# koadman/libMems

Measured on AMD Instinct MI355X. Metric: seed-mers/sec sorted+matched (+ MUMs/sec) at 1/2/4/8 MI355X; HBM GB/s vs roofline, higher is better.
Workload: dtype u64; 1 GPU; BASELINE config 3: 8 x 100 Mbp, seed weight 19 (0x7b974ef), MemHash seed stage (sorted+matched); genomes=8, genome_length=100000000, seedmers_total=799999792, seedmers_rank0=799999792, probes_rank0=100459493, parallelism=1 GPU

## Files before the change

libmems_amd/csrc/groups.hip:

```cpp
#include <cstdlib>
#include <type_traits>

#include "match_device.h"
#include "seed_device.h"

namespace mums {

namespace {

constexpr int kGTile = kSegTile;
constexpr int kGRounds = kGTile / kBlock;
constexpr int kSlots = kGTile / 2;
#ifndef MUMS_GROUP_SPLIT
#define MUMS_GROUP_SPLIT 2
#endif
constexpr int kGSplit = MUMS_GROUP_SPLIT;
constexpr int kGSub = kGTile / kGSplit;
constexpr int kGSubRounds = kGSub / kBlock;
constexpr int kSubSlots = kGSub / 2;
static_assert(kGSub % kBlock == 0 && kGSubRounds * (kBlock / 64) <= 64, "probe sub-tile");

__device__ __forceinline__ uint32_t blk_excl_scan(uint32_t v, uint32_t* s_w, uint32_t* total) {
    const int lane = threadIdx.x & 63, wv = threadIdx.x >> 6;
    uint32_t inc = v;
    #pragma unroll
    for (int d = 1; d < 64; d <<= 1) {
        uint32_t t = __shfl_up(inc, d, 64);
        if (lane >= d) inc += t;
    }
    if (lane == 63) s_w[wv] = inc;
    __syncthreads();
// ... 134 lines not shown
                                                                double inv_table) {
    constexpr int kGRounds = kGSubRounds;
    constexpr int kWaves = kBlock / 64;
    __shared__ uint64_t srec[kGSub];
    __shared__ uint16_t heads[kSubSlots];
    __shared__ uint32_t wcnt[kGRounds * kWaves];
    __shared__ uint32_t s_w[2][kWaves];
    __shared__ uint32_t s_ng[kWaves];
    __shared__ uint32_t s_red[2];
    __shared__ uint64_t s_prev, s_next;
    __shared__ uint8_t s_gl[256];
    __shared__ uint32_t s_gb[kMaxG + 1];
    const int lane = threadIdx.x & 63;
    const int wv = __builtin_amdgcn_readfirstlane(threadIdx.x >> 6);
    const SegTile td = tiles[blockIdx.x / kGSplit];
    const uint32_t part0 = (blockIdx.x % kGSplit) * (uint32_t)kGSub;
    if (td.count <= part0) {
        if (threadIdx.x == 0) {
            tile_count[blockIdx.x] = 0;
            tile_count[gridDim.x + 32 + blockIdx.x] = 0;
        }
        return;
    }
    const uint64_t tile0 = td.start + part0;
    const uint32_t cnt = td.count - part0 < (uint32_t)kGSub ? td.count - part0 : (uint32_t)kGSub;

    uint32_t kx[kGRounds];
    {
        uint64_t x[kGRounds];
        #pragma unroll
        for (int r = 0; r < kGRounds; ++r) {
            const uint32_t q = r * kBlock + threadIdx.x;
            x[r] = rec[tile0 + (q < cnt ? q : cnt - 1)];
        }
        #pragma unroll
        for (int r = 0; r < kGRounds; ++r) {
            const uint32_t q = r * kBlock + threadIdx.x;
            if (q < cnt) srec[q] = x[r];
            kx[r] = (uint32_t)(x[r] >> (IB + 1));
        }
// ... 137 lines not shown
                                                               const uint32_t* __restrict__ tile_off,
                                                               const uint64_t* __restrict__ slot_info,
                                                               const uint32_t* __restrict__ slot_bucket,
                                                               uint64_t* __restrict__ probe_info,
                                                               uint32_t* __restrict__ probe_bucket,
                                                               uint32_t slots_per_block) {
    const uint32_t n = tile_count[blockIdx.x];
    const uint64_t o = tile_off[blockIdx.x];
    const uint64_t sb = (uint64_t)blockIdx.x * slots_per_block;
    for (uint32_t k = threadIdx.x; k < n; k += kBlock) {
        probe_info[o + k] = slot_info[sb + k];
        probe_bucket[o + k] = slot_bucket[sb + k];
    }
}

__global__ void flat_tiles_kernel(uint64_t N, uint64_t nt, SegTile* __restrict__ tiles) {
    const uint64_t t = (uint64_t)blockIdx.x * blockDim.x + threadIdx.x;
    if (t >= nt) return;
    SegTile d{};
    d.start = t * kGTile;
    d.bstart = 0;
    d.bend = N;
    const uint64_t rem = N - d.start;
    d.count = (uint32_t)(rem < (uint64_t)kGTile ? rem : (uint64_t)kGTile);
    d.hbase = 0;
    d.ntb = (uint32_t)nt;
    d.tb = (uint32_t)t;
    tiles[t] = d;
}

#ifndef MUMS_MAT_WIDE
#define MUMS_MAT_WIDE 1
#endif
constexpr bool kMatWide = MUMS_MAT_WIDE != 0;
struct __attribute__((aligned(8))) Rec2 { uint64_t a, b; };

template <int MG, typename View, bool kGl = false>
__global__ __launch_bounds__(kBlock) void probe_materialize_kernel(View v, const uint64_t* __restrict__ probe_info,
                                                                   uint64_t P, GenomeTable gt, MatchParams mp, int L,
// ... 356 lines not shown
    hipLaunchKernelGGL(row_bucket_kernel, dim3((unsigned)((P + kBlock - 1) / kBlock)), dim3(kBlock), 0, st, rows, P, G,
                       table_size, 1.0 / (double)table_size, d_bounds, nranks, out);
    return hipGetLastError();
}

hipError_t launch_gather_rows(const int64_t* src, const uint32_t* perm, uint64_t P, int G, int64_t* dst,
                              hipStream_t st) {
    if (P == 0) return hipSuccess;
    const uint64_t n = P * (uint64_t)(G + 1);
    const uint64_t per = (uint64_t)kBlock * kGatherIPT;
    hipLaunchKernelGGL(gather_rows_ilp_kernel, dim3((unsigned)((n + per - 1) / per)), dim3(kBlock), 0, st, src, perm, n,
                       (uint32_t)(G + 1), dst);
    return hipGetLastError();
}

hipError_t launch_flat_tiles(uint64_t N, SegTile* d_tiles, hipStream_t st) {
    const uint64_t nt = (N + kGTile - 1) / kGTile;
    if (nt == 0) return hipSuccess;
    hipLaunchKernelGGL(flat_tiles_kernel, dim3((unsigned)((nt + 255) / 256)), dim3(256), 0, st, N, nt, d_tiles);
    return hipGetLastError();
}

template <int MG, typename View>
hipError_t launch_probe_tiles(View v, const SegTile* tiles, uint64_t ntiles, uint64_t N, const GenomeTable& gt,
                              const MatchParams& mp, int L, uint32_t* tile_count, uint64_t* slot_info,
                              uint32_t* slot_bucket, void* counters, hipStream_t st) {
    if (ntiles == 0) return hipSuccess;
    if constexpr (RecIB<View>::value > 0) {
        const bool fast = mp.repeat_tol == 0 && mp.enum_tol == 1;
        const double inv_t = 1.0 / (double)mp.table_size;
        if (RecIB<View>::value == 32 && gt.gl_n > 0 && fast && !getenv("MUMS_DEV_PROBE_GENERAL"))
            hipLaunchKernelGGL((probe_tile_rec_kernel<MG, RecIB<View>::value, true, true>),
                               dim3((unsigned)(ntiles * kGSplit)), dim3(kBlock), 0, st, v.rec, tiles, gt, mp, L,
                               tile_count, slot_info, slot_bucket, (DevCounters*)counters, inv_t);
// ... 74 lines not shown
```

libmems_amd/csrc/mums_capi.hip:

```cpp
#include <hip/hip_runtime.h>

#include <algorithm>
#include <array>
#include <chrono>
#include <functional>
#include <cstddef>
#include <cstdio>
#include <cstdlib>
#include <cstring>
#include <memory>
#include <string>
#include <vector>

#include "../../include/mums.h"
#include "match_device.h"
#include "mums_internal.h"
#include "seed_device.h"

using namespace mums;

namespace {

struct DevBuf {
    void* p = nullptr;
// ... 767 lines not shown
        HIPCHK(ctx->ctab.ensure(64));
        HIPCHK(hipMemsetAsync(ctx->ctab.p, 0, 64, st));
        HIPCHK(launch_seed_scatter_chunk(ctx->ss, lgt, ctx->packed.as<uint32_t>(), B, hist, T, 0, 0, out, st,
                                         ctx->ctab.as<uint64_t>(), B));
    }
    HIPCHK(seg_bucket_starts(B > 0 ? hist : nullptr, T, B, n, bstart, st));
    return MUMS_OK;
}

void records_live(mums_ctx* ctx) {
    for (DevBuf* b : {&ctx->rowtmp, &ctx->sids, &ctx->summ, &ctx->chain_tmp}) b->drop_view();
}

int ensure_merge_space(mums_ctx* ctx, uint64_t n, int mb, int key_bits, ProbeSpace* ps) {
    records_live(ctx);
    const uint64_t ub = seg_tiles_upper(n, mb);
    HIPCHK(ctx->recA.ensure(n * 8 + 64));
    HIPCHK(ctx->recB.ensure(n * 8 + 64));
    HIPCHK(ctx->tiles.ensure(ub * sizeof(SegTile) + 64));
    HIPCHK(ctx->mstart.ensure(((1ull << mb) + 64) * 4));
    size_t tmpb = std::max(seg_tmp_bytes(n, mb), onesweep_tmp_bytes(n, mb, key_bits));
    tmpb = std::max(tmpb, std::max(scan_tmp_bytes(n), radix_tmp_bytes(n / 2 + 1)));
    tmpb = std::max(tmpb, scan_tmp_bytes((uint64_t)ctx->table_size));
    HIPCHK(ctx->tmp.ensure(tmpb));
    return ensure_probe_space(ctx, n, ub, ps);
}

int tie_fix_stream(mums_ctx* ctx, const RsStream& s, uint64_t n, hipStream_t st);
bool wants_tie_order(const mums_ctx* ctx);

int merge_stage(mums_ctx* ctx, uint64_t n, int mb, int key_bits, const MatchParams& mp, const ProbeSpace& ps,
                hipStream_t st, int ib = 32, uint64_t* rA = nullptr, uint64_t* rB = nullptr) {
    DevCounters* dc = ctx->counters.as<DevCounters>();
    if (!rA) rA = ctx->recA.as<uint64_t>();
    if (!rB) rB = ctx->recB.as<uint64_t>();
    SegTile* tiles = ctx->tiles.as<SegTile>();
    const uint32_t* bstart = ctx->mstart.as<uint32_t>();
    const uint64_t ub = seg_tiles_upper(n, mb);
    const bool prof = ctx->profiling;
    HIPCHK(build_seg_tiles_from_starts(bstart, mb, n, tiles, &dc->ntiles, ctx->tmp.p, st));
    int buf = 0;
    if (ib != 32 && !(n < (1ull << 30) && key_bits <= 32))
        return fail(ctx, MUMS_E_UNSUPPORTED, "33-bit records need < 2^30 records per merge");
    const bool mask_parity = mp.repeat_tol == 0 && mp.enum_tol == 1;
    ctx->parity_masked = false;
    const bool onesweep = ctx->use_onesweep && n < (1ull << 30) && key_bits <= 32;
    const bool wide = onesweep && mask_parity && ib == 32 && seg_wide_sort_enabled() && seg_wide_passes(key_bits) <= 3;
    if (wide) {
        HIPCHK(seg_onesweep_sort_wide(rA, rB, n, key_bits, mb, bstart, ctx->tmp.p, &dc->err, &buf, st,
                                      prof ? ctx->ev_ds : nullptr, 32));
        ctx->parity_masked = true;
    } else if (onesweep) {
        HIPCHK(seg_onesweep_sort(rA, rB, n, key_bits, mb, bstart, ctx->tmp.p, &dc->err, &buf, st,
                                 prof ? ctx->ev_ds : nullptr, ib, mask_parity));
        ctx->parity_masked = mask_parity && seg_onesweep_launches(key_bits) < (key_bits + 7) / 8;
    } else
        HIPCHK(seg_radix_sort(rA, rB, n, key_bits, tiles, ub, ctx->tmp.p, &buf, st, prof ? ctx->ev_ds : nullptr));
    ctx->sorted_buf = buf;
    ctx->sorted_rec = buf ? rB : rA;
    ctx->sort_passes = wide ? seg_wide_passes(key_bits) : onesweep ? seg_onesweep_launches(key_bits) : (key_bits + 7) / 8;
    HIPCHK(hipEventRecord(ctx->ev[EV_SORT], st));
    if (wants_tie_order(ctx) && ib == 32 && !ctx->shard) {
        RsStream s{};
        s.kind = 0;
        s.rec = ctx->sorted_rec;
        s.bstart = bstart;
        s.B = mb;
        s.kbits = 2 * ctx->w + 1;
        const int rc = tie_fix_stream(ctx, s, n, st);
        if (rc) return rc;
    }
    if (ib == 33)
// ... 273 lines not shown
        s.B = B;
        s.kbits = 2 * ctx->w + 1;
        uint64_t* dst = ctx->sorted_buf ? ctx->recA.as<uint64_t>() : ctx->recB.as<uint64_t>();
        if (ctx->parity_masked) {
            HIPCHK(seg_parity_fix(const_cast<uint64_t*>(ctx->sorted_rec), dst, N, s.kbits - B, B, ctx->mstart.as<uint32_t>(), ctx->tmp.p,
                                  &dc->err, st));
            ctx->parity_masked = false;
        }
        HIPCHK(ctx->rsbst.ensure(((1ull << B) + 64) * 4));
        rc = restart_fixup(ctx, s, N, dst, nullptr, ctx->rsbst.as<uint32_t>(), &nl, &changed, st);
        if (rc || !changed) return rc;
        HIPCHK(hipMemcpyAsync(ctx->mstart.p, ctx->rsbst.p, ((1ull << B) + 1) * 4, hipMemcpyDeviceToDevice, st));
        ctx->sorted_buf ^= 1;
        ctx->sorted_rec = dst;
        SegTile* tiles = ctx->tiles.as<SegTile>();
        HIPCHK(build_seg_tiles_from_starts(ctx->mstart.as<uint32_t>(), B, nl, tiles, &dc->ntiles, ctx->tmp.p, st));
        HIPCHK(hipMemsetAsync(&dc->repeat_limit, 0, 8, st));
        rc = groups_dispatch<RecView>(ctx, RecView{dst}, tiles, seg_tiles_upper(nl, B), mp, ps.probe_info,
                                      ps.probe_bucket, ps.slot_info, ps.slot_bucket, st);
    } else {
        const size_t kb = ctx->key64 ? 8 : 4;
        (void)kb;
        s.kind = ctx->key64 ? 2 : 1;
        s.key = ctx->sorted_key;
        s.idx = ctx->sorted_idx;
        void* dk = ctx->sorted_buf ? ctx->kA.p : ctx->kB.p;
        uint32_t* dv = ctx->sorted_buf ? ctx->vA.as<uint32_t>() : ctx->vB.as<uint32_t>();
        rc = restart_fixup(ctx, s, N, dk, dv, nullptr, &nl, &changed, st);
        if (rc || !changed) return rc;
        ctx->sorted_buf ^= 1;
        ctx->sorted_key = dk;
        ctx->sorted_idx = dv;
        SegTile* tiles = ctx->tiles.as<SegTile>();
// ... 327 lines not shown
    const int kbits = 2 * ctx->w + 1;
    int gbits = 0;
    while ((1 << gbits) < G) ++gbits;
    if (kbits + gbits > 63) return fail(ctx, MUMS_E_UNSUPPORTED, "ParallelMemHash compat: seed weight too large");
    ctx->packed_path = false;
    ctx->key64 = true;
    ctx->msd_bits = 0;
    ctx->progress.clear();
    const uint64_t kmask = (1ull << kbits) - 1;

    uint64_t words = 0;
    const uint32_t T = layout_packed(gt, &words);
    HIPCHK(ctx->packed.ensure(words * 4 + 64));
    HIPCHK(ctx->counters.ensure(sizeof(DevCounters)));
    DevCounters* dc = ctx->counters.as<DevCounters>();
    const uint64_t ntiles_groups = (N + kSegTile - 1) / kSegTile;
    HIPCHK(ctx->ckey.ensure(N * 8 + 64));
    HIPCHK(ctx->kA.ensure(N * 8 + 64));
    HIPCHK(ctx->kB.ensure(N * 8 + 64));
    HIPCHK(ctx->vA.ensure(N * 4 + 64));
    HIPCHK(ctx->vB.ensure(N * 4 + 64));
    HIPCHK(ctx->cval.ensure(enum_rows ? 2 * (N + 64) * 4 : N * 4 + 64));
    HIPCHK(ctx->tiles.ensure(ntiles_groups * sizeof(SegTile) + 64));
    size_t tmpb = std::max(scan_tmp_bytes(N + 1), radix_tmp_bytes(N + 1));
    tmpb = std::max(tmpb, scan_tmp_bytes((uint64_t)ctx->table_size));
    HIPCHK(ctx->tmp.ensure(tmpb));
    ProbeSpace ps{};
    int rc = ensure_probe_space(ctx, N, ntiles_groups, &ps);
    if (rc) return rc;

    int mx = -1;
// ... 263 lines not shown
        HIPCHK(hipEventRecord(ctx->ev[EV_BUCKETS], st));
        ctx->stage_done = MUMS_STAGE_SEEDS;
        if (stage >= MUMS_STAGE_ALL) {
            rc = find_tail(ctx, mp, ctx->packed.as<uint32_t>(), [&](MatProbes* v) {
                v->rows = ctx->mprobe.as<int64_t>();
                return MUMS_OK;
            }, st);
            if (rc) return rc;
        }
        HIPCHK(hipStreamSynchronize(st));
        HIPCHK(hipMemcpy(&ctx->hc, dc, sizeof(DevCounters), hipMemcpyDeviceToHost));
        fill_stats(ctx, N);
        return MUMS_OK;
    }
    SegTile* tiles = ctx->tiles.as<SegTile>();
    HIPCHK(launch_flat_tiles(n_live, tiles, st));
    if (ctx->compat_rec)
        rc = groups_dispatch<RecView>(ctx, RecView{ctx->sorted_rec}, tiles, (n_live + kSegTile - 1) / kSegTile, mp,
                                      ps.probe_info, ps.probe_bucket, ps.slot_info, ps.slot_bucket, st);
    else
        rc = groups_dispatch<PairView<uint64_t>>(
            ctx, PairView<uint64_t>{(const uint64_t*)ctx->sorted_key, ctx->sorted_idx}, tiles,
            (n_live + kSegTile - 1) / kSegTile, mp, ps.probe_info, ps.probe_bucket, ps.slot_info, ps.slot_bucket, st);
    if (rc) return rc;
    rc = finish_seeds(ctx, ps, st, stage >= MUMS_STAGE_ALL);
    if (rc) return rc;
    ctx->compat_pfirst.clear();
    if (ctx->match_log) {
        DevBuf pf;
        HIPCHK(pf.ensure(((uint64_t)nch + 1) * 4 + 64));
        HIPCHK(launch_compat_probe_chunks(ctx->probe_info, ctx->P, (const uint64_t*)ctx->sorted_key, kbits, nch,
                                          pf.as<uint32_t>(), st));
        ctx->compat_pfirst.resize((size_t)nch + 1);
// ... 148 lines not shown
    if (!s) return fail(ctx, MUMS_E_INVALID, "null stream");
    if (ctx->own_stream && ctx->stream) (void)hipStreamDestroy(ctx->stream);
    ctx->stream = (hipStream_t)s;
    ctx->own_stream = false;
    return MUMS_OK;
}

int mums_set_seed(mums_ctx* ctx, uint64_t pattern) {
    if (check_ctx(ctx)) return MUMS_E_INVALID;
    ctx->seed = pattern;
    return MUMS_OK;
}

int mums_set_params(mums_ctx* ctx, uint32_t repeat_tol, uint32_t enum_tol, uint32_t table_size) {
    if (check_ctx(ctx)) return MUMS_E_INVALID;
    if (table_size == 0 || table_size > 0x7FFFFFFFu)
        return fail(ctx, MUMS_E_INVALID, "table size must be in [1, 2^31)");
    ctx->repeat_tol = repeat_tol;
    ctx->enum_tol = enum_tol;
    ctx->table_size = table_size;
    return MUMS_OK;
}

int mums_set_mask(mums_ctx* ctx, int masked, uint64_t seq_mask) {
    if (check_ctx(ctx)) return MUMS_E_INVALID;
    ctx->masked = masked ? 1 : 0;
    ctx->seq_mask = seq_mask;
    return MUMS_OK;
}

int mums_add_genome(mums_ctx* ctx, const char* ascii, uint64_t n) {
    if (check_ctx(ctx)) return MUMS_E_INVALID;
// ... 853 lines not shown
    const auto chunks = shard_key_chunks(bst, ctx->shard_kcount, shard_chunk_cap());
    if (chunks.empty() && ctx->shard_kcount)
        return fail(ctx, MUMS_E_UNSUPPORTED, "one MSD bucket holds more than 2^30 records");
    DevCounters* dc = ctx->counters.as<DevCounters>();
    const MatchParams mp{ctx->repeat_tol, ctx->enum_tol, ctx->table_size, ctx->masked, ctx->seq_mask};
    const size_t W = (size_t)(G + 1) * 8;
    uint64_t P_total = 0, groups = 0;
    ctx->fused_keys = false;
    for (const auto& ch : chunks) {
        const uint32_t b0 = ch.first, b1 = ch.second;
        const uint64_t o = bst[b0], nc = (uint64_t)bst[b1] - o;
        std::vector<uint32_t> sub(nbk + 1);
        for (uint32_t b = 0; b <= nbk; ++b) sub[b] = b < b0 ? 0u : (b < b1 ? bst[b] - (uint32_t)o : (uint32_t)nc);
        HIPCHK(hipMemcpyAsync(ctx->mstart.p, sub.data(), sub.size() * 4, hipMemcpyHostToDevice, st));
        SegTile* tiles = ctx->tiles.as<SegTile>();
        HIPCHK(build_seg_tiles_from_starts(ctx->mstart.as<uint32_t>(), mb, nc, tiles, &dc->ntiles, ctx->tmp.p, st));
        const uint64_t ub = seg_tiles_upper(nc, mb);
        int rc;
        if (ctx->rec_ib == 33)
            rc = groups_dispatch<RecViewT<33>>(ctx, RecViewT<33>{rec + o}, tiles, ub, mp, ps.probe_info,
                                               ps.probe_bucket, ps.slot_info, ps.slot_bucket, st);
        else
            rc = groups_dispatch<RecView>(ctx, RecView{rec + o}, tiles, ub, mp, ps.probe_info, ps.probe_bucket,
                                          ps.slot_info, ps.slot_bucket, st);
        if (rc) return rc;
        rc = finish_seeds(ctx, ps, st);
        if (rc) return rc;
        const uint64_t Pc = ctx->P;
        if (rows && Pc) {
            if (P_total + Pc >= (1ull << 32) - 64)
                return fail(ctx, MUMS_E_UNSUPPORTED, "more than 2^32 seed probes on one rank");
            if (ctx->rowsall.cap < (P_total + Pc + 1) * W) {
// ... 63 lines not shown
    if (pw && ib33) HIPCHK(launch_pairwise_emit(v64, n, ctx->gt, ctx->L, ncalls, off, rows, st));
    else if (pw) HIPCHK(launch_pairwise_emit(v, n, ctx->gt, ctx->L, ncalls, off, rows, st));
    else if (ib33) HIPCHK(launch_enum_emit(v64, n, ctx->gt, mp, ctx->L, ncalls, off, P, rows, st));
    else HIPCHK(launch_enum_emit(v, n, ctx->gt, mp, ctx->L, ncalls, off, P, rows, st));
    HIPCHK(hipStreamSynchronize(st));
    ctx->P = P;
    ctx->st.probes = P;
    ctx->shard_rows_built = true;
    return MUMS_OK;
}

int shard_chunk_rows(mums_ctx* ctx, hipStream_t st) {
    if (!shard_rows_from_all(ctx) || ctx->shard_rows_built) return MUMS_OK;
    if (ctx->enum_tol > 1 || ctx->pairwise) return shard_enum_rows(ctx, st);
    ProbeSpace ps{};
    int rc = ensure_probe_space(ctx, ctx->shard_n, seg_tiles_upper(ctx->shard_n, ctx->shard_mb), &ps);
    if (rc) return rc;
    HIPCHK(hipMemsetAsync(ctx->counters.p, 0, sizeof(DevCounters), st));
    rc = shard_groups_chunked(ctx, const_cast<uint64_t*>(ctx->sorted_rec), ctx->shard_bst, ps, true, st);
    if (rc) return rc;
    ctx->shard_rows_built = true;
    return MUMS_OK;
}

int shard_regroup(mums_ctx* ctx, uint64_t* dst, uint64_t nl, const std::vector<uint32_t>& bst, const ProbeSpace& ps,
                  uint64_t restarts, const uint64_t* offset_log, hipStream_t st) {
    const int mb = ctx->shard_mb;
    ctx->sorted_buf ^= 1;
    ctx->sorted_rec = dst;
    DevCounters* dc = ctx->counters.as<DevCounters>();
    const uint64_t rep = ctx->hc.repeat_limit;
// ... 9 lines not shown
        const uint64_t P = ctx->P, groups = ctx->st.groups;
        ctx->hc.repeat_limit = rep;
        ctx->restarts = restarts;
        ctx->offset_log.assign(offset_log, offset_log + restarts * (uint64_t)ctx->gt.G);
        ctx->shard_restart_pending = false;
        shard_merge_stats(ctx, nl);
        ctx->P = P;
        ctx->st.probes = P;
        ctx->st.groups = groups;
        return MUMS_OK;
    }
    HIPCHK(hipMemcpyAsync(ctx->mstart.p, bst.data(), bst.size() * 4, hipMemcpyHostToDevice, st));
    ctx->live_n = nl;
    ctx->live_bst = bst;
    SegTile* tiles = ctx->tiles.as<SegTile>();
    HIPCHK(build_seg_tiles_from_starts(ctx->mstart.as<uint32_t>(), mb, nl, tiles, &dc->ntiles, ctx->tmp.p, st));
    HIPCHK(hipMemsetAsync(&dc->repeat_limit, 0, 8, st));
    const MatchParams mp{ctx->repeat_tol, ctx->enum_tol, ctx->table_size, ctx->masked, ctx->seq_mask};
    const uint64_t ub = seg_tiles_upper(nl, mb);
    int rc;
    if (ctx->rec_ib == 33)
        rc = groups_dispatch<RecViewT<33>>(ctx, RecViewT<33>{dst}, tiles, ub, mp, ps.probe_info, ps.probe_bucket,
                                           ps.slot_info, ps.slot_bucket, st);
    else
        rc = groups_dispatch<RecView>(ctx, RecView{dst}, tiles, ub, mp, ps.probe_info, ps.probe_bucket, ps.slot_info,
                                      ps.slot_bucket, st);
    if (rc) return rc;
    rc = finish_seeds(ctx, ps, st);
    if (rc) return rc;
    HIPCHK(h2d_sync(&dc->repeat_limit, &rep, 8, ctx->stream));
    ctx->hc.repeat_limit = rep;
    ctx->restarts = restarts;
    ctx->offset_log.assign(offset_log, offset_log + restarts * (uint64_t)ctx->gt.G);
    ctx->shard_restart_pending = false;
// ... 1780 lines not shown
        HIPCHK(hipEventRecord(ctx->ev[EV_CHAINS], st));
        uint32_t* bstart = ctx->mstart.as<uint32_t>();
        if (!resident) {
            HIPCHK(exclusive_scan_u32(slice, (uint64_t)nbc8 * T, ctx->tmp.p, nullptr, st));
            HIPCHK(launch_seed_scatter_chunk(ctx->ss, gt, ctx->packed.as<uint32_t>(), B, slice, T, dlo, nbc8, rA, st));
        }
        if (live_rec) {
            n_c = n_live[c];
            HIPCHK(hipMemcpyAsync(bstart, lbst.as<uint32_t>() + (uint64_t)c * (nbc + 1), (nbc + 1) * 4ull,
                                  hipMemcpyDeviceToDevice, st));
        } else {
            rc = chunk_starts(c, n_c, bstart);
            if (rc) return rc;
        }
        SegTile* tiles = ctx->tiles.as<SegTile>();
        const uint64_t ub = seg_tiles_upper(n_c, mb);
        HIPCHK(build_seg_tiles_from_starts(bstart, mb, n_c, tiles, &dc->ntiles, ctx->tmp.p, st));
        if (!resident) {
            int buf = 0;
            HIPCHK(seg_onesweep_sort(rA, rB, n_c, 31, mb, bstart, ctx->tmp.p, &dc->err, &buf, st,
                                     prof ? ctx->ev_ds : nullptr, 33, mp.repeat_tol == 0 && mp.enum_tol == 1));
            ctx->sorted_rec = buf ? rB : rA;
            if (prof)
                for (int p = 0; p < npass; ++p) {
                    float ms = 0.f;
                    (void)hipEventElapsedTime(&ms, ctx->ev_ds[2 * p], ctx->ev_ds[2 * p + 1]);
                    ms_dom += ms;
                }
            dom_bytes += n_c * 16 * (uint64_t)npass;
            dom_launches += (uint64_t)npass;
        } else {
            ctx->sorted_rec = live_rec ? live_rec + o : (sbuf ? rB : rA);
// ... 646 lines not shown
```

libmems_amd/csrc/mums_internal.h:

```cpp
#pragma once

#include <hip/hip_runtime.h>
#include <stdint.h>
#include <stdlib.h>

#include <vector>

#include "restart_plan.h"

namespace mums {

constexpr int kMaxG = 64;
constexpr int kRepeatLimit = 1000;
constexpr int kBlock = 256;
#ifndef MUMS_SEED_TILE
#define MUMS_SEED_TILE 4096
#endif
constexpr int kSeedTile = MUMS_SEED_TILE;
#ifndef MUMS_SEG_TILE
#define MUMS_SEG_TILE 4096
#endif
constexpr int kSegTile = MUMS_SEG_TILE;
constexpr int kLocalIPT = 16;
constexpr int kMaxMsdBits = 11;
constexpr int kMaxSegBucketBits = 12;

constexpr int kMaxSeedRuns = 16;

struct SeedSpec {
    uint64_t pattern;
    int L;
    int w;
    int nruns;
    int run_start[32];
    int run_len[32];
    int run_dst[32];
    int run_sh[kMaxSeedRuns];
// ... 158 lines not shown
                             const uint32_t* d_bstart, void* d_tmp, uint32_t* d_err, int* out_buf, hipStream_t st,
                             hipEvent_t* ev_ds = nullptr, int key_shift = 32, bool mask_parity = false,
                             bool key_runs = false, const uint32_t* hist_in = nullptr,
                             const uint64_t* gsrc = nullptr, uint32_t* gout = nullptr);
size_t seg_parity_fix_tmp_bytes(uint64_t n);
hipError_t seg_parity_fix(uint64_t* rec, uint64_t* scratch, uint64_t n, int key_bits, int msd_bits,
                          const uint32_t* d_bstart, void* d_tmp, uint32_t* d_err, hipStream_t st, int key_shift = 32);
int seg_onesweep_launches(int key_bits);
bool seg_wide_sort_enabled();
int seg_wide_passes(int key_bits);
size_t onesweep_wide_tmp_bytes(uint64_t n, int msd_bits, int key_bits);
hipError_t seg_onesweep_sort_wide(uint64_t* recA, uint64_t* recB, uint64_t n, int key_bits, int msd_bits,
                                  const uint32_t* d_bstart, void* d_tmp, uint32_t* d_err, int* out_buf,
                                  hipStream_t st, hipEvent_t* ev_ds, int key_shift = 32);

uint64_t group_slot_count(uint64_t ntiles);
uint64_t group_blocks(uint64_t ntiles, bool packed);
template <int MG, typename View>
hipError_t launch_probe_tiles(View v, const SegTile* tiles, uint64_t ntiles, uint64_t N, const GenomeTable& gt,
                              const MatchParams& mp, int L, uint32_t* tile_count, uint64_t* slot_info,
                              uint32_t* slot_bucket, void* counters, hipStream_t st);
hipError_t launch_probe_compact(uint64_t nblocks, const uint32_t* tile_count, const uint32_t* tile_off,
                                const uint64_t* slot_info, const uint32_t* slot_bucket, uint64_t* probe_info,
                                uint32_t* probe_bucket, hipStream_t st, bool packed);
hipError_t launch_bucket_records(const uint32_t* b, uint64_t P, uint64_t* rec, hipStream_t st);
hipError_t launch_bucket_split(const uint64_t* rec, uint64_t P, uint32_t* b, uint32_t* ids, hipStream_t st);
template <int MG, typename View>
hipError_t launch_materialize(View v, const uint64_t* probe_info, uint64_t P, const GenomeTable& gt,
                              const MatchParams& mp, int L, int64_t* rows, hipStream_t st, uint64_t* lkey = nullptr,
                              uint32_t* fsk = nullptr, uint32_t* lhash = nullptr, int32_t* rows32 = nullptr);
// ... 7 lines not shown
                              int kb_rec, uint64_t* key, uint64_t* idx, hipStream_t st);
hipError_t launch_chain_dest(const uint32_t* fk, uint64_t nch, const uint32_t* pdest, uint32_t* cdest, hipStream_t st);
hipError_t launch_inverse_perm(const uint32_t* perm, uint64_t n, uint32_t* inv, hipStream_t st);
hipError_t launch_chain_tags(const uint32_t* chain_of, const uint32_t* perm, const uint32_t* sdest, uint64_t P,
                             const uint32_t* cinv, const uint32_t* cstart, uint32_t* tags, hipStream_t st);
hipError_t launch_chain_entries_out(const int64_t* pool, const uint32_t* fk, const uint32_t* cperm,
                                    const uint32_t* scdest, uint64_t nch, int G, const uint32_t* pinv,
                                    const uint32_t* rstart, int64_t* eout, uint32_t* fout, hipStream_t st);
hipError_t launch_kept_dest(const int64_t* rows, uint64_t P, int G, const uint32_t* chain_of, const uint32_t* cinv,
                            const uint2* thr, const uint32_t* fk, const uint32_t* pdest, uint32_t nranks, uint32_t* dest,
                            hipStream_t st);
hipError_t launch_dest_first(const uint32_t* sdest, uint64_t P, uint32_t* first, hipStream_t st);
hipError_t launch_entry_first(const uint32_t* scdest, uint64_t nch, const uint32_t* rcount, const uint32_t* perm,
                              const uint32_t* sdest, uint64_t K, const uint32_t* chain_of, const uint32_t* cinv,
                              const uint32_t* rstart, uint32_t* efirst, hipStream_t st);
hipError_t launch_flat_tiles(uint64_t N, SegTile* d_tiles, hipStream_t st);

hipError_t launch_bucket_ranges(const uint32_t* sb, uint64_t P, uint32_t* bstart, uint32_t* bend, uint32_t* d_max,
                                hipStream_t st);
template <int MG, typename View>
hipError_t launch_replay_kept(View v, const GenomeTable& gt, const MatchParams& mp, int L, uint64_t P,
                              const int64_t* pool, const uint32_t* chain_of, const uint32_t* fk, uint32_t nch,
                              void* d_tmp, void* d_radix_tmp, void* d_scan_tmp, uint32_t lds_cap, uint32_t* tsize,
                              void* ctr, uint64_t* dbg, hipStream_t st, uint64_t* mlog, uint32_t** tbl_out,
                              const uint32_t** base_out, void* (*alloc)(void*, size_t), void* alloc_ctx,
                              const uint32_t* jl = nullptr);
}
struct mums_ctx;
namespace mums {
hipStream_t ctx_stream(mums_ctx* ctx);
int ctx_device(mums_ctx* ctx);
// ... 256 lines not shown
```

libmems_amd/csrc/seed_device.h:

```cpp
#pragma once

#include "mums_internal.h"

namespace mums {

__device__ __forceinline__ uint32_t xcd_grouped_block(uint32_t b, uint32_t n) {
    const uint32_t q = n >> 3, r = n & 7u, x = b & 7u;
    return (x < r ? x * (q + 1) : r * (q + 1) + (x - r) * q) + (b >> 3);
}

__device__ __forceinline__ uint64_t revcomp2w(uint64_t v, int w) {
    uint64_t x = ~v;
    x = __builtin_bitreverse64(x);
    x = ((x >> 1) & 0x5555555555555555ull) | ((x & 0x5555555555555555ull) << 1);
    return x >> (64 - 2 * w);
}

__device__ __forceinline__ uint64_t ckey_finish(uint64_t v, int w) {
    const uint64_t rc = revcomp2w(v, w);
    const uint64_t par = rc < v ? 1ull : 0ull;
    return ((par ? rc : v) << 1) | par;
}

__device__ __forceinline__ uint64_t ckey_from_mer(uint64_t mer, const SeedSpec& ss) {
// ... 60 lines not shown
__device__ __forceinline__ uint32_t ckey_top_static(uint64_t mer) {
    constexpr SeedRuns R = seed_runs(PAT);
    constexpr int B = (K + 1) / 2;
    static_assert(K >= 1 && 2 * B <= 2 * R.w && 2 * B <= 32, "top digit wider than the seed");
    uint64_t v = 0;
    #pragma unroll
    for (int r = 0; r < R.n; ++r) v |= (R.sh[r] >= 0 ? (mer >> R.sh[r]) : (mer << -R.sh[r])) & R.mask[r];
    const uint32_t ft = (uint32_t)(v >> (2 * R.w - K));
    const uint32_t lowc = ~(uint32_t)v & (uint32_t)((1ull << (2 * B)) - 1);
    uint32_t rr = __builtin_bitreverse32(lowc) >> (32 - 2 * B);
    rr = ((rr >> 1) & 0x55555555u) | ((rr & 0x55555555u) << 1);
    const uint32_t rt = rr >> (2 * B - K);
    return ft < rt ? ft : rt;
}

constexpr uint64_t kSeedW15 = 0x7ac9afull;
constexpr uint64_t kSeedW19 = 0x7b974efull;
constexpr uint64_t kSeedW21 = 0x7ddaddfull;

__device__ __forceinline__ uint64_t window_at(const uint32_t* __restrict__ W, uint64_t p) {
    const uint64_t wi = p >> 4;
    const int sh = 2 * (int)(p & 15);
    const uint64_t hi = ((uint64_t)W[wi] << 32) | W[wi + 1];
    const uint64_t lo = W[wi + 2];
    return (hi << sh) | ((lo << sh) >> 32);
}

__device__ __forceinline__ uint64_t ckey_at(const uint32_t* __restrict__ W, uint64_t p, const SeedSpec& ss) {
    return ckey_from_mer(window_at(W, p), ss);
}
// ... 41 lines not shown
```

libmems_amd/csrc/seeds.hip:

```cpp
#include <cstdlib>
#include <type_traits>

#include "seed_device.h"

namespace mums {

namespace {

constexpr int kTile = kSeedTile;
constexpr int kPerThread = kTile / kBlock;
constexpr int kHalo = 32;
constexpr int kTileBytes = kTile + kHalo;
constexpr int kTileWords = kTileBytes / 16 + 3;
constexpr int kWaves = kBlock / 64;

struct AsciiPtrs { const char* p[kMaxG]; };

template <uint64_t PAT>
constexpr int kStaticMsd = PAT == 0 ? 0 : (2 * seed_runs(PAT).w + 1 > 32 ? 2 * seed_runs(PAT).w + 1 - 32 : 0);

__device__ __forceinline__ uint32_t dna2(uint32_t c) {
    const uint32_t lc = c | 0x20u;
    const uint32_t one = (lc == 'c') | (lc == 'b') | (lc == 'y');
    const uint32_t two = (lc == 'g') | (lc == 's') | (lc == 'k');
// ... 91 lines not shown
    {
        const uint64_t pw = packed_words(n);
        uint32_t* out = packed + gt.woff[g];
        for (int k = tid; k < kTile / 16 + 2; k += kBlock) {
            const uint64_t wi = (uint64_t)x * (kTile / 16) + k;
            if ((k < kTile / 16 || p0 + kTile >= n) && wi < pw) out[wi] = words[k];
        }
    }

    if (kMode == 1 && nb <= 1) return;
    const uint64_t base = gt.base[g];
    const int klow = 2 * ss.w + 1 - msd_bits;
    if constexpr (kMode == 1 && PAT != 0 && kStaticMsd<PAT> >= 1 && kStaticMsd<PAT> <= kMaxMsdBits) {
        constexpr int kTop = kStaticMsd<PAT> > 8 ? 8 : kStaticMsd<PAT>;
        if (msd_bits == kTop) {
            #pragma unroll 4
            for (int j = 0; j < kPerThread; ++j) {
                const int q = tid + j * kBlock;
                const uint64_t p = p0 + (uint64_t)q;
                if (p >= m) break;
                const int wi = q >> 4, sh = 2 * (q & 15);
                const uint64_t hi = ((uint64_t)words[wi] << 32) | words[wi + 1];
                const uint64_t lo = words[wi + 2];
                atomicAdd(&bh[ckey_top_static<PAT, kTop>((hi << sh) | ((lo << sh) >> 32))], 1u);
            }
            __syncthreads();
            for (int i = tid; i < nb; i += kBlock) hist[(uint64_t)i * T + t] = bh[i];
            return;
        }
    }
// ... 369 lines not shown
```

Baseline: 37.32 billion seed-mers/s.

## Decouple probe tile take from staging size and add register-field top-key histogram

Probe workgroups now consume a configurable slice (kProbeTake, default 1984) rather than the full staged half-tile. Tile builders, upper bounds and flat tiles take a separate probe tile size, and the radix-sort path rebuilds sort-sized tiles before rebuilding probe tiles. A new specialized MSD histogram path extracts the top-bit canonical key from two 32-bit register fields using alignbit per thread, processing 16 contiguous positions per thread instead of strided word loads. The aim is less per-seed extraction work in the histogram and better probe-tile balance and occupancy, at the cost of more tiles, extra tile rebuilds and layout-dependent correctness risk. The table size bound is also relaxed to allow 2^31.

```diff
diff --git a/libmems_amd/csrc/groups.hip b/libmems_amd/csrc/groups.hip
--- a/libmems_amd/csrc/groups.hip
+++ b/libmems_amd/csrc/groups.hip
@@ -11,10 +11,8 @@
 constexpr int kGTile = kSegTile;
 constexpr int kGRounds = kGTile / kBlock;
 constexpr int kSlots = kGTile / 2;
-#ifndef MUMS_GROUP_SPLIT
-#define MUMS_GROUP_SPLIT 2
-#endif
-constexpr int kGSplit = MUMS_GROUP_SPLIT;
+constexpr int kGSplit = kProbeSplit;
+constexpr int kGTake = kProbeTake;
 constexpr int kGSub = kGTile / kGSplit;
 constexpr int kGSubRounds = kGSub / kBlock;
 constexpr int kSubSlots = kGSub / 2;
@@ -179,7 +177,7 @@
     const int lane = threadIdx.x & 63;
     const int wv = __builtin_amdgcn_readfirstlane(threadIdx.x >> 6);
     const SegTile td = tiles[blockIdx.x / kGSplit];
-    const uint32_t part0 = (blockIdx.x % kGSplit) * (uint32_t)kGSub;
+    const uint32_t part0 = (blockIdx.x % kGSplit) * (uint32_t)kGTake;
     if (td.count <= part0) {
         if (threadIdx.x == 0) {
             tile_count[blockIdx.x] = 0;
@@ -188,7 +186,7 @@
         return;
     }
     const uint64_t tile0 = td.start + part0;
-    const uint32_t cnt = td.count - part0 < (uint32_t)kGSub ? td.count - part0 : (uint32_t)kGSub;
+    const uint32_t cnt = td.count - part0 < (uint32_t)kGTake ? td.count - part0 : (uint32_t)kGTake;
 
     uint32_t kx[kGRounds];
     {
@@ -356,15 +354,15 @@
     }
 }
 
-__global__ void flat_tiles_kernel(uint64_t N, uint64_t nt, SegTile* __restrict__ tiles) {
+__global__ void flat_tiles_kernel(uint64_t N, uint64_t nt, uint32_t tile, SegTile* __restrict__ tiles) {
     const uint64_t t = (uint64_t)blockIdx.x * blockDim.x + threadIdx.x;
     if (t >= nt) return;
     SegTile d{};
-    d.start = t * kGTile;
+    d.start = t * tile;
     d.bstart = 0;
     d.bend = N;
     const uint64_t rem = N - d.start;
-    d.count = (uint32_t)(rem < (uint64_t)kGTile ? rem : (uint64_t)kGTile);
+    d.count = (uint32_t)(rem < (uint64_t)tile ? rem : (uint64_t)tile);
     d.hbase = 0;
     d.ntb = (uint32_t)nt;
     d.tb = (uint32_t)t;
@@ -751,10 +749,11 @@
     return hipGetLastError();
 }
 
-hipError_t launch_flat_tiles(uint64_t N, SegTile* d_tiles, hipStream_t st) {
-    const uint64_t nt = (N + kGTile - 1) / kGTile;
+hipError_t launch_flat_tiles(uint64_t N, SegTile* d_tiles, hipStream_t st, bool packed) {
+    const uint32_t tile = (uint32_t)(packed ? kProbeTile : kGTile);
+    const uint64_t nt = (N + tile - 1) / tile;
     if (nt == 0) return hipSuccess;
-    hipLaunchKernelGGL(flat_tiles_kernel, dim3((unsigned)((nt + 255) / 256)), dim3(256), 0, st, N, nt, d_tiles);
+    hipLaunchKernelGGL(flat_tiles_kernel, dim3((unsigned)((nt + 255) / 256)), dim3(256), 0, st, N, nt, tile, d_tiles);
     return hipGetLastError();
 }
 
diff --git a/libmems_amd/csrc/mums_capi.hip b/libmems_amd/csrc/mums_capi.hip
--- a/libmems_amd/csrc/mums_capi.hip
+++ b/libmems_amd/csrc/mums_capi.hip
@@ -805,7 +805,7 @@
 
 int ensure_merge_space(mums_ctx* ctx, uint64_t n, int mb, int key_bits, ProbeSpace* ps) {
     records_live(ctx);
-    const uint64_t ub = seg_tiles_upper(n, mb);
+    const uint64_t ub = group_tiles_upper(n, mb);
     HIPCHK(ctx->recA.ensure(n * 8 + 64));
     HIPCHK(ctx->recB.ensure(n * 8 + 64));
     HIPCHK(ctx->tiles.ensure(ub * sizeof(SegTile) + 64));
@@ -827,9 +827,9 @@
     if (!rB) rB = ctx->recB.as<uint64_t>();
     SegTile* tiles = ctx->tiles.as<SegTile>();
     const uint32_t* bstart = ctx->mstart.as<uint32_t>();
-    const uint64_t ub = seg_tiles_upper(n, mb);
+    const uint64_t ub = group_tiles_upper(n, mb);
     const bool prof = ctx->profiling;
-    HIPCHK(build_seg_tiles_from_starts(bstart, mb, n, tiles, &dc->ntiles, ctx->tmp.p, st));
+    HIPCHK(build_seg_tiles_from_starts(bstart, mb, n, tiles, &dc->ntiles, ctx->tmp.p, st, kProbeTile));
     int buf = 0;
     if (ib != 32 && !(n < (1ull << 30) && key_bits <= 32))
         return fail(ctx, MUMS_E_UNSUPPORTED, "33-bit records need < 2^30 records per merge");
@@ -845,8 +845,12 @@
         HIPCHK(seg_onesweep_sort(rA, rB, n, key_bits, mb, bstart, ctx->tmp.p, &dc->err, &buf, st,
                                  prof ? ctx->ev_ds : nullptr, ib, mask_parity));
         ctx->parity_masked = mask_parity && seg_onesweep_launches(key_bits) < (key_bits + 7) / 8;
-    } else
-        HIPCHK(seg_radix_sort(rA, rB, n, key_bits, tiles, ub, ctx->tmp.p, &buf, st, prof ? ctx->ev_ds : nullptr));
+    } else {
+        HIPCHK(build_seg_tiles_from_starts(bstart, mb, n, tiles, &dc->ntiles, ctx->tmp.p, st));
+        HIPCHK(seg_radix_sort(rA, rB, n, key_bits, tiles, seg_tiles_upper(n, mb), ctx->tmp.p, &buf, st,
+                              prof ? ctx->ev_ds : nullptr));
+        HIPCHK(build_seg_tiles_from_starts(bstart, mb, n, tiles, &dc->ntiles, ctx->tmp.p, st, kProbeTile));
+    }
     ctx->sorted_buf = buf;
     ctx->sorted_rec = buf ? rB : rA;
     ctx->sort_passes = wide ? seg_wide_passes(key_bits) : onesweep ? seg_onesweep_launches(key_bits) : (key_bits + 7) / 8;
@@ -1150,9 +1154,10 @@
         ctx->sorted_buf ^= 1;
         ctx->sorted_rec = dst;
         SegTile* tiles = ctx->tiles.as<SegTile>();
-        HIPCHK(build_seg_tiles_from_starts(ctx->mstart.as<uint32_t>(), B, nl, tiles, &dc->ntiles, ctx->tmp.p, st));
+        HIPCHK(build_seg_tiles_from_starts(ctx->mstart.as<uint32_t>(), B, nl, tiles, &dc->ntiles, ctx->tmp.p, st,
+                                           kProbeTile));
         HIPCHK(hipMemsetAsync(&dc->repeat_limit, 0, 8, st));
-        rc = groups_dispatch<RecView>(ctx, RecView{dst}, tiles, seg_tiles_upper(nl, B), mp, ps.probe_info,
+        rc = groups_dispatch<RecView>(ctx, RecView{dst}, tiles, group_tiles_upper(nl, B), mp, ps.probe_info,
                                       ps.probe_bucket, ps.slot_info, ps.slot_bucket, st);
     } else {
         const size_t kb = ctx->key64 ? 8 : 4;
@@ -1510,7 +1515,7 @@
     HIPCHK(ctx->packed.ensure(words * 4 + 64));
     HIPCHK(ctx->counters.ensure(sizeof(DevCounters)));
     DevCounters* dc = ctx->counters.as<DevCounters>();
-    const uint64_t ntiles_groups = (N + kSegTile - 1) / kSegTile;
+    const uint64_t ntiles_groups = flat_group_tiles(N, true);
     HIPCHK(ctx->ckey.ensure(N * 8 + 64));
     HIPCHK(ctx->kA.ensure(N * 8 + 64));
     HIPCHK(ctx->kB.ensure(N * 8 + 64));
@@ -1804,9 +1809,9 @@
         return MUMS_OK;
     }
     SegTile* tiles = ctx->tiles.as<SegTile>();
-    HIPCHK(launch_flat_tiles(n_live, tiles, st));
+    HIPCHK(launch_flat_tiles(n_live, tiles, st, ctx->compat_rec));
     if (ctx->compat_rec)
-        rc = groups_dispatch<RecView>(ctx, RecView{ctx->sorted_rec}, tiles, (n_live + kSegTile - 1) / kSegTile, mp,
+        rc = groups_dispatch<RecView>(ctx, RecView{ctx->sorted_rec}, tiles, flat_group_tiles(n_live, true), mp,
                                       ps.probe_info, ps.probe_bucket, ps.slot_info, ps.slot_bucket, st);
     else
         rc = groups_dispatch<PairView<uint64_t>>(
@@ -1985,8 +1990,8 @@
 
 int mums_set_params(mums_ctx* ctx, uint32_t repeat_tol, uint32_t enum_tol, uint32_t table_size) {
     if (check_ctx(ctx)) return MUMS_E_INVALID;
-    if (table_size == 0 || table_size > 0x7FFFFFFFu)
-        return fail(ctx, MUMS_E_INVALID, "table size must be in [1, 2^31)");
+    if (table_size == 0 || table_size > 0x80000000u)
+        return fail(ctx, MUMS_E_INVALID, "table size must be in [1, 2^31]");
     ctx->repeat_tol = repeat_tol;
     ctx->enum_tol = enum_tol;
     ctx->table_size = table_size;
@@ -2870,8 +2875,9 @@
         for (uint32_t b = 0; b <= nbk; ++b) sub[b] = b < b0 ? 0u : (b < b1 ? bst[b] - (uint32_t)o : (uint32_t)nc);
         HIPCHK(hipMemcpyAsync(ctx->mstart.p, sub.data(), sub.size() * 4, hipMemcpyHostToDevice, st));
         SegTile* tiles = ctx->tiles.as<SegTile>();
-        HIPCHK(build_seg_tiles_from_starts(ctx->mstart.as<uint32_t>(), mb, nc, tiles, &dc->ntiles, ctx->tmp.p, st));
-        const uint64_t ub = seg_tiles_upper(nc, mb);
+        HIPCHK(build_seg_tiles_from_starts(ctx->mstart.as<uint32_t>(), mb, nc, tiles, &dc->ntiles, ctx->tmp.p, st,
+                                           kProbeTile));
+        const uint64_t ub = group_tiles_upper(nc, mb);
         int rc;
         if (ctx->rec_ib == 33)
             rc = groups_dispatch<RecViewT<33>>(ctx, RecViewT<33>{rec + o}, tiles, ub, mp, ps.probe_info,
@@ -2965,7 +2971,7 @@
     if (!shard_rows_from_all(ctx) || ctx->shard_rows_built) return MUMS_OK;
     if (ctx->enum_tol > 1 || ctx->pairwise) return shard_enum_rows(ctx, st);
     ProbeSpace ps{};
-    int rc = ensure_probe_space(ctx, ctx->shard_n, seg_tiles_upper(ctx->shard_n, ctx->shard_mb), &ps);
+    int rc = ensure_probe_space(ctx, ctx->shard_n, group_tiles_upper(ctx->shard_n, ctx->shard_mb), &ps);
     if (rc) return rc;
     HIPCHK(hipMemsetAsync(ctx->counters.p, 0, sizeof(DevCounters), st));
     rc = shard_groups_chunked(ctx, const_cast<uint64_t*>(ctx->sorted_rec), ctx->shard_bst, ps, true, st);
@@ -3005,10 +3011,11 @@
     ctx->live_n = nl;
     ctx->live_bst = bst;
     SegTile* tiles = ctx->tiles.as<SegTile>();
-    HIPCHK(build_seg_tiles_from_starts(ctx->mstart.as<uint32_t>(), mb, nl, tiles, &dc->ntiles, ctx->tmp.p, st));
+    HIPCHK(build_seg_tiles_from_starts(ctx->mstart.as<uint32_t>(), mb, nl, tiles, &dc->ntiles, ctx->tmp.p, st,
+                                       kProbeTile));
     HIPCHK(hipMemsetAsync(&dc->repeat_limit, 0, 8, st));
     const MatchParams mp{ctx->repeat_tol, ctx->enum_tol, ctx->table_size, ctx->masked, ctx->seq_mask};
-    const uint64_t ub = seg_tiles_upper(nl, mb);
+    const uint64_t ub = group_tiles_upper(nl, mb);
     int rc;
     if (ctx->rec_ib == 33)
         rc = groups_dispatch<RecViewT<33>>(ctx, RecViewT<33>{dst}, tiles, ub, mp, ps.probe_info, ps.probe_bucket,
@@ -4819,8 +4826,8 @@
             if (rc) return rc;
         }
         SegTile* tiles = ctx->tiles.as<SegTile>();
-        const uint64_t ub = seg_tiles_upper(n_c, mb);
-        HIPCHK(build_seg_tiles_from_starts(bstart, mb, n_c, tiles, &dc->ntiles, ctx->tmp.p, st));
+        const uint64_t ub = group_tiles_upper(n_c, mb);
+        HIPCHK(build_seg_tiles_from_starts(bstart, mb, n_c, tiles, &dc->ntiles, ctx->tmp.p, st, kProbeTile));
         if (!resident) {
             int buf = 0;
             HIPCHK(seg_onesweep_sort(rA, rB, n_c, 31, mb, bstart, ctx->tmp.p, &dc->err, &buf, st,
diff --git a/libmems_amd/csrc/mums_internal.h b/libmems_amd/csrc/mums_internal.h
--- a/libmems_amd/csrc/mums_internal.h
+++ b/libmems_amd/csrc/mums_internal.h
@@ -21,6 +21,17 @@
 #define MUMS_SEG_TILE 4096
 #endif
 constexpr int kSegTile = MUMS_SEG_TILE;
+#ifndef MUMS_GROUP_SPLIT
+#define MUMS_GROUP_SPLIT 2
+#endif
+#ifndef MUMS_PROBE_TAKE
+#define MUMS_PROBE_TAKE 1984
+#endif
+constexpr int kProbeSplit = MUMS_GROUP_SPLIT;
+constexpr int kProbeTake = MUMS_PROBE_TAKE;
+constexpr int kProbeTile = kProbeSplit * kProbeTake;
+static_assert(kSegTile % kProbeSplit == 0 && kProbeTake >= 2 && kProbeTake <= kSegTile / kProbeSplit,
+              "a probe workgroup takes at most what it stages");
 constexpr int kLocalIPT = 16;
 constexpr int kMaxMsdBits = 11;
 constexpr int kMaxSegBucketBits = 12;
@@ -209,6 +220,7 @@
                                   const uint32_t* d_bstart, void* d_tmp, uint32_t* d_err, int* out_buf,
                                   hipStream_t st, hipEvent_t* ev_ds, int key_shift = 32);
 
+inline uint64_t group_tiles_upper(uint64_t n, int msd_bits) { return seg_tiles_upper(n, msd_bits, kProbeTile); }
 uint64_t group_slot_count(uint64_t ntiles);
 uint64_t group_blocks(uint64_t ntiles, bool packed);
 template <int MG, typename View>
@@ -246,7 +258,11 @@
 hipError_t launch_entry_first(const uint32_t* scdest, uint64_t nch, const uint32_t* rcount, const uint32_t* perm,
                               const uint32_t* sdest, uint64_t K, const uint32_t* chain_of, const uint32_t* cinv,
                               const uint32_t* rstart, uint32_t* efirst, hipStream_t st);
-hipError_t launch_flat_tiles(uint64_t N, SegTile* d_tiles, hipStream_t st);
+hipError_t launch_flat_tiles(uint64_t N, SegTile* d_tiles, hipStream_t st, bool packed = false);
+inline uint64_t flat_group_tiles(uint64_t N, bool packed) {
+    const uint64_t tile = packed ? kProbeTile : kSegTile;
+    return (N + tile - 1) / tile;
+}
 
 hipError_t launch_bucket_ranges(const uint32_t* sb, uint64_t P, uint32_t* bstart, uint32_t* bend, uint32_t* d_max,
                                 hipStream_t st);
diff --git a/libmems_amd/csrc/seed_device.h b/libmems_amd/csrc/seed_device.h
--- a/libmems_amd/csrc/seed_device.h
+++ b/libmems_amd/csrc/seed_device.h
@@ -98,6 +98,69 @@
     return ft < rt ? ft : rt;
 }
 
+struct TopRuns {
+    int nh = 0, nt = 0, hspan = 0, tspan = 0, toff = 0;
+    int hsh[16] = {}, tsh[16] = {};
+    uint32_t hmask[16] = {}, tmask[16] = {};
+};
+
+constexpr TopRuns top_runs(uint64_t pat, int B) {
+    TopRuns T{};
+    const SeedRuns R = seed_runs(pat);
+    if (B < 1 || B > 16 || B > R.w) return T;
+    int c = 0;
+    for (int k = 0; k < R.L && c < B; ++k) {
+        if (!((pat >> (R.L - 1 - k)) & 1)) continue;
+        T.hspan = k + 1;
+        if (k < 16) {
+            const int dst = 2 * (B - 1 - c), sh = (30 - 2 * k) - dst;
+            if (T.nh > 0 && T.hsh[T.nh - 1] == sh) T.hmask[T.nh - 1] |= 3u << dst;
+            else { T.hsh[T.nh] = sh; T.hmask[T.nh] = 3u << dst; ++T.nh; }
+        }
+        ++c;
+    }
+    c = 0;
+    for (int k = R.L - 1; k >= 0 && c < B; --k) {
+        if (!((pat >> (R.L - 1 - k)) & 1)) continue;
+        T.toff = k;
+        ++c;
+    }
+    T.tspan = R.L - T.toff;
+    c = 0;
+    for (int k = R.L - 1; k >= 0 && c < B; --k) {
+        if (!((pat >> (R.L - 1 - k)) & 1)) continue;
+        if (k - T.toff < 16) {
+            const int dst = 2 * c, sh = (30 - 2 * (k - T.toff)) - dst;
+            if (T.nt > 0 && T.tsh[T.nt - 1] == sh) T.tmask[T.nt - 1] |= 3u << dst;
+            else { T.tsh[T.nt] = sh; T.tmask[T.nt] = 3u << dst; ++T.nt; }
+        }
+        ++c;
+    }
+    return T;
+}
+
+template <uint64_t PAT, int K>
+constexpr bool kTopFields = PAT != 0 && top_runs(PAT, (K + 1) / 2).nh > 0 && top_runs(PAT, (K + 1) / 2).hspan <= 16 &&
+                            top_runs(PAT, (K + 1) / 2).tspan <= 16;
+
+template <uint64_t PAT, int K>
+__device__ __forceinline__ uint32_t ckey_top_fields(uint32_t head, uint32_t tail) {
+    constexpr int B = (K + 1) / 2;
+    constexpr TopRuns T = top_runs(PAT, B);
+    static_assert(kTopFields<PAT, K>, "head or tail wider than one field");
+    uint32_t hv = 0, tv = 0;
+    #pragma unroll
+    for (int r = 0; r < T.nh; ++r) hv |= (T.hsh[r] >= 0 ? (head >> T.hsh[r]) : (head << -T.hsh[r])) & T.hmask[r];
+    #pragma unroll
+    for (int r = 0; r < T.nt; ++r) tv |= (T.tsh[r] >= 0 ? (tail >> T.tsh[r]) : (tail << -T.tsh[r])) & T.tmask[r];
+    const uint32_t ft = hv >> (2 * B - K);
+    const uint32_t lowc = ~tv & (uint32_t)((1ull << (2 * B)) - 1);
+    uint32_t rr = __builtin_bitreverse32(lowc) >> (32 - 2 * B);
+    rr = ((rr >> 1) & 0x55555555u) | ((rr & 0x55555555u) << 1);
+    const uint32_t rt = rr >> (2 * B - K);
+    return ft < rt ? ft : rt;
+}
+
 constexpr uint64_t kSeedW15 = 0x7ac9afull;
 constexpr uint64_t kSeedW19 = 0x7b974efull;
 constexpr uint64_t kSeedW21 = 0x7ddaddfull;
diff --git a/libmems_amd/csrc/seeds.hip b/libmems_amd/csrc/seeds.hip
--- a/libmems_amd/csrc/seeds.hip
+++ b/libmems_amd/csrc/seeds.hip
@@ -129,6 +129,22 @@
     if constexpr (kMode == 1 && PAT != 0 && kStaticMsd<PAT> >= 1 && kStaticMsd<PAT> <= kMaxMsdBits) {
         constexpr int kTop = kStaticMsd<PAT> > 8 ? 8 : kStaticMsd<PAT>;
         if (msd_bits == kTop) {
+            if constexpr (kTopFields<PAT, kTop> && seed_runs(PAT).L <= kHalo + 1 && kPerThread == 16) {
+                constexpr int kToff = top_runs(PAT, (kTop + 1) / 2).toff;
+                const uint32_t w[4] = {words[tid], words[tid + 1], words[tid + 2], 0u};
+                const uint64_t q0 = p0 + (uint64_t)tid * 16;
+                const int rem = q0 >= m ? 0 : (m - q0 < 16 ? (int)(m - q0) : 16);
+                #pragma unroll
+                for (int j = 0; j < 16; ++j) {
+                    const int a = (j + kToff) >> 4, s = (j + kToff) & 15;
+                    const uint32_t head = j == 0 ? w[0] : __builtin_amdgcn_alignbit(w[0], w[1], 32 - 2 * j);
+                    const uint32_t tail = s == 0 ? w[a] : __builtin_amdgcn_alignbit(w[a], w[a + 1], 32 - 2 * s);
+                    if (j < rem) atomicAdd(&bh[ckey_top_fields<PAT, kTop>(head, tail)], 1u);
+                }
+                __syncthreads();
+                for (int i = tid; i < nb; i += kBlock) hist[(uint64_t)i * T + t] = bh[i];
+                return;
+            }
             #pragma unroll 4
             for (int j = 0; j < kPerThread; ++j) {
                 const int q = tid + j * kBlock;
```

Result: faster. 37.98 billion seed-mers/s (median of 6 runs) (+1.8%).
